# rpng/suo_slam

Measured on AMD Instinct MI355X. Metric: frames/sec (obj-crops/sec) YCB-V 640x480 8-obj; ADD(-S) vs ref, higher is better.
Workload: dtype f32 (2 x fp16 split products)

## Files before the change

### suo_slam_amd/build.py

```python
from __future__ import annotations

import os
import subprocess
import sys

HERE = os.path.dirname(os.path.abspath(__file__))
CSRC = os.path.join(HERE, "csrc")
LIB = os.path.join(HERE, "libsuo_hip.so")
SOURCES = ["capi.hip", "net.hip", "net_weights.hip", "conv.hip", "conv_wino.hip", "conv_wino_x3.hip", "conv_wino_x3_dma.hip", "conv_wino_x3_skip_dma.hip", "conv_small.hip", "stem_x3.hip", "res_small.hip", "res_small_x3.hip", "gemm_persist.hip", "gemm_bf16x3.hip", "misc.hip", "calibrate.hip", "pnp.hip", "lm.hip", "lm_big.hip", "lm_cam.hip", "lm_cam2.hip", "lm_frame.hip", "lm_frame2.hip", "lm_dist.hip", "pose_cov.hip", "pose_cov_graph.hip", "resid_stats.hip", "track_cov.hip", "ba_comm.hip", "pnp_api.hip", "ba_stage.hip", "ba_api.hip", "ba_ctx.hip", "ba_drive.hip", "cov_stage.hip", "pose_cov_api.hip", "track_cov_api.hip", "frame_geom.hip", "eval.hip", "eval_bop.hip", "eval_points.hip", "eval_nees.hip", "eval_nees_api.hip", "raster.hip", "eval_vsd.hip", "gt_info.hip", "gt_info_api.hip", "eval_masks.hip", "slam_score.hip", "slam_vote.hip", "viz.hip", "viz_api.hip"]
HIPCC = os.environ.get("HIPCC", "/opt/rocm/bin/hipcc")
FLAGS = ["--offload-arch=gfx950", "-O3", "-std=c++17", "-fPIC", "-ffp-contract=off"]


def _stale(target, deps):
    if not os.path.exists(target):
        return True
    t = os.path.getmtime(target)
    return any(os.path.getmtime(d) > t for d in deps)


def build(force: bool = False, verbose: bool = True) -> str:
    srcs = [os.path.join(CSRC, s) for s in SOURCES if os.path.exists(os.path.join(CSRC, s))]
    hdrs = [os.path.join(CSRC, f) for f in os.listdir(CSRC) if f.endswith(".h")]
    hdrs.append(os.path.join(os.path.dirname(HERE), "include", "suo_hip.h"))
    objs = []
    procs = []
    for src in srcs:
        obj = src[:-4] + ".o"
        objs.append(obj)
        deps = [src] + hdrs
        if src.endswith("lm_big.hip"):
            deps.append(os.path.join(CSRC, "lm.hip"))
        if force or _stale(obj, deps):
            cmd = [HIPCC] + FLAGS + ["-c", src, "-o", obj]
            if verbose:
                print(" ".join(cmd), flush=True)
            procs.append((src, subprocess.Popen(cmd)))
    for src, p in procs:
        if p.wait() != 0:
            raise RuntimeError(f"hipcc failed on {src}")
    if force or procs or _stale(LIB, objs):
        cmd = [HIPCC, "--offload-arch=gfx950", "-shared", "-fPIC", "-o", LIB] + objs + ["-ldl"]
        if verbose:
            print(" ".join(cmd), flush=True)
        subprocess.check_call(cmd)
    return LIB


if __name__ == "__main__":
    build(force="--force" in sys.argv)
    print(LIB)
```

### suo_slam_amd/csrc/conv_wino_x3_dma.hip

```cpp
#include "conv_wino_x3_kernel.h"

namespace suo {

int launch_conv3x3_wino_f16x2_dma(const ConvArgs& a, hipStream_t s, int tiles) {
    if (a.N == 64) hipLaunchKernelGGL((wino3x3_x3_kernel<false, false, false, 2, 2, false, false, false, true>), dim3(tiles), dim3(256), 0, s, a);
    else hipLaunchKernelGGL((wino3x3_x3_kernel<false, false, false, 4, 2, false, false, false, true>), dim3(tiles), dim3(256), 0, s, a);
    SUO_HIP_CHECK(hipGetLastError());
    return SUO_OK;
}
int launch_conv3x3_wino_f16x2_fused_dma(const ConvArgs& a, hipStream_t s, int tiles) {
    if (a.n_W1) hipLaunchKernelGGL((wino3x3_x3_kernel<true, false, true, 4, 2, true, false, false, true>), dim3(tiles), dim3(256), 0, s, a);
    else if (a.up) hipLaunchKernelGGL((wino3x3_x3_kernel<true, true, true, 4, 2, false, false, false, true>), dim3(tiles), dim3(256), 0, s, a);
    else hipLaunchKernelGGL((wino3x3_x3_kernel<true, false, true, 4, 2, false, false, false, true>), dim3(tiles), dim3(256), 0, s, a);
    SUO_HIP_CHECK(hipGetLastError());
    return SUO_OK;
}

}
```

### suo_slam_amd/csrc/conv_wino_x3_kernel.h

```cpp
#pragma once
#include <string.h>

#include "buffer_ops.h"
#include "mma_ops.h"
#include "suo_internal.h"
#include "tune.h"

namespace suo {

__device__ __forceinline__ f32x4 x_sub4(f32x4 a, f32x4 b) { return a - b; }
__device__ __forceinline__ f32x4 x_add4(f32x4 a, f32x4 b) { return a + b; }
__device__ __forceinline__ void x_add16(f32x16& z, const f32x16& t) { z += t; }
__device__ __forceinline__ void x_sub16(f32x16& z, const f32x16& t) { z -= t; }

constexpr int X_CK = 16, X_PKH = 20, X_TH = 8, X_TW = 16, X_IH = 10, X_IW = 18, X_NPIX = X_IH * X_IW;

template <bool FUSE, bool UP = false, bool TX3 = false, int NT = 4, int NP = 3, bool NEXT = false, bool SKD = false, bool W8 = false, bool DMA = false>
__global__ __launch_bounds__(W8 ? 512 : 256) __attribute__((amdgpu_waves_per_eu(2))) void wino3x3_x3_kernel(const ConvArgs a) {
    static_assert(NT == 4 || (NT == 2 && !FUSE), "64-channel form: plain convolution only");
    static_assert(!DMA || (NP == 2 && !W8), "halo by LDS-DMA: the four-wave fp16 form");
    static_assert(!SKD || (DMA && FUSE && TX3 && UP && !NEXT), "skip rows by LDS-DMA: the LDS-DMA form's tail with the up-sampled addend (the form it measured faster on)");
    static_assert(!W8 || (NT == 4 && NP == 2 && !NEXT && (TX3 || !FUSE)), "eight waves: the fp16 form of the 128-channel kernel, without the next block's conv1");
    constexpr int NTHR = W8 ? 512 : 256;
    static_assert(!NEXT || (FUSE && TX3 && NP == 2), "the next block's conv1 rides on the fp16 tail");
    static_assert(NP == 3 || !FUSE || TX3, "the fp16 form's tail runs on the fp16 pipe");
    constexpr int HSZ = X_NPIX * X_PKH;
    constexpr int VROW = 16;
    constexpr int VPL = 16 * 32 * VROW;
    constexpr int VFLOATS = NP * VPL / 2;
    constexpr int TAILF = NP * 8 * (64 * 32 + 32) / 4;
    constexpr int SKF = SKD ? 4 * 1024 : 0;
    constexpr int SFLOATS = W8 ? (2 * HSZ + VFLOATS > TAILF + 8 * 32 * 36 ? 2 * HSZ + VFLOATS : TAILF + 8 * 32 * 36) : 2 * HSZ + VFLOATS + SKF;
    static_assert(SFLOATS * 4 <= 80 * 1024, "two workgroups per CU");
    __shared__ __attribute__((aligned(16))) float S[SFLOATS];
    float (*Hin)[HSZ] = reinterpret_cast<float (*)[HSZ]>(&S[0]);
    uint16_t* V = reinterpret_cast<uint16_t*>(&S[2 * HSZ]);
    const int tid = threadIdx.x, lane = tid & 63;
    const int w = __builtin_amdgcn_readfirstlane(tid >> 6);
    const int tiles_x = (a.OW + X_TW - 1) / X_TW, tiles_y = (a.OH + X_TH - 1) / X_TH;
    int bid = xcd_block_id();
    const int l = bid / (tiles_x * tiles_y);
    bid -= l * tiles_x * tiles_y;
    const int ty0 = bid / tiles_x, tx0 = bid - ty0 * tiles_x;
    const int oy0 = ty0 * X_TH, ox0 = tx0 * X_TW;
    const int iy0 = oy0 - 1, ix0 = ox0 - 1;
    const int nch = a.C / X_CK;
    const float* in_l = a.in + (size_t)l * a.H * a.W * a.C;
    const __amdgpu_buffer_rsrc_t in_srd = make_srd(in_l, (size_t)a.H * a.W * a.C * sizeof(float));
    const __amdgpu_buffer_rsrc_t w_srd = make_srd(a.Wp, (size_t)a.N * a.C * 16 * NP * sizeof(uint16_t));
    const __amdgpu_buffer_rsrc_t out_srd = make_srd(a.out + (size_t)l * a.OH * a.OW * a.N, (size_t)a.OH * a.OW * a.N * sizeof(float));

    constexpr int NF4 = X_NPIX * 4, NLD = (NF4 + NTHR - 1) / NTHR;
    constexpr int HP = DMA ? 16 : X_PKH;
    static_assert(!DMA || (NLD == 3 && NLD * NTHR * 4 <= HSZ), "LDS-DMA staging: three 1 KiB pieces per wave inside a halo buffer");
    int avoff[NLD];
#pragma unroll
    for (int i = 0; i < NLD; ++i) {
        const int idx = tid + i * NTHR;
        const int pix = idx >> 2;
        const int py = pix / X_IW, px = pix - py * X_IW;
        const int cc = DMA ? (idx & 3) ^ ((py >> 1) & 3) : idx & 3;
        const int iy = iy0 + py, ix = ix0 + px;
        const bool ok = idx < NF4 && iy >= 0 && iy < a.H && ix >= 0 && ix < a.W;
        avoff[i] = ok ? ((iy * a.W + ix) * a.C + cc * 4) * 4 : BUF_OOB;
    }
    const unsigned lds_w = __builtin_amdgcn_readfirstlane((unsigned)(size_t)&S[0]) + w * 1024;
    auto dma = [&](int c, int buf) {
        if constexpr (DMA) {
            const unsigned d0 = lds_w + buf * (HSZ * 4), d1 = d0 + NTHR * 16, d2 = d0 + 2 * NTHR * 16;
            const int soff = c * X_CK * 4;
            unsigned keep;
            asm volatile("s_mov_b32 %0, m0\n\t"
                         "s_nop 4\n\t"
                         "s_mov_b32 m0, %5\n\ts_nop 0\n\tbuffer_load_dwordx4 %1, %4, %8 offen lds\n\t"
                         "s_mov_b32 m0, %6\n\ts_nop 0\n\tbuffer_load_dwordx4 %2, %4, %8 offen lds\n\t"
                         "s_mov_b32 m0, %7\n\ts_nop 0\n\tbuffer_load_dwordx4 %3, %4, %8 offen lds\n\t"
                         "s_mov_b32 m0, %0"
                         : "=&s"(keep)
                         : "v"(avoff[0]), "v"(avoff[NLD > 1 ? 1 : 0]), "v"(avoff[NLD > 2 ? 2 : 0]), "s"(in_srd), "s"(d0), "s"(d1), "s"(d2), "s"(soff)
                         : "memory");
        }
    };
    f32x4 areg[NLD];
    auto gload = [&](int c) {
#pragma unroll
        for (int i = 0; i < NLD; ++i) areg[i] = buf_load(in_srd, avoff[i], c * X_CK * 4);
    };
    float dmax = 0.f;
    const float xs = NP == 2 ? s2_xscale(a.xscale) : 1.f;
    auto sstore = [&](int buf) {
#pragma unroll
        for (int i = 0; i < NLD; ++i) {
            const int idx = tid + i * NTHR;
            if constexpr (NP == 2) {
                areg[i] *= xs;
                dmax = s2_track(s2_track(dmax, areg[i][0], areg[i][1]), areg[i][2], areg[i][3]);
            }
            if (idx < NF4) *(f32x4*)&Hin[buf][(idx >> 2) * X_PKH + (idx & 3) * 4] = areg[i];
        }
    };
    auto dtrack = [&](int buf) {
#pragma unroll
        for (int i = 0; i < NLD; ++i) {
            const f32x4 v = *(const f32x4*)&Hin[buf][(tid + i * NTHR) * 4];
            dmax = s2_track(s2_track(dmax, v[0], v[1]), v[2], v[3]);
        }
    };
    const int wvoff = lane * 16;
    const int wn = NT == 4 ? (W8 ? (w & 3) : w) : (w & 1), wc = NT == 4 ? (W8 ? (w >> 2) : 0) : (w >> 1);
    constexpr bool HALF = NT == 2 || W8;
    constexpr int NPAIR = HALF ? 4 : 8;
    const int wsbase = wn * NP * 1024;
    auto bload = [&](int gc, u32x4 (&b)[NP]) {
        const int g = gc;
#pragma unroll
        for (int p = 0; p < NP; ++p) b[p] = __builtin_bit_cast(u32x4, buf_load(w_srd, wvoff + p * 1024, g * (NT * NP * 1024) + wsbase));
    };
    const int tt = tid & 31, tq = (tid >> 5) & 3, th = (tid >> 7) & 1;
    const int tv = __builtin_amdgcn_readfirstlane(tid >> 8);
    const int t_ty = tt >> 3, t_tx = tt & 7;
    const int hbase = ((2 * t_ty + th) * X_IW + 2 * t_tx) * HP + (DMA ? (tq ^ t_ty) : tq) * 4;
    const int hbase1 = DMA ? ((2 * t_ty + th) * X_IW + 2 * t_tx) * HP + (tq ^ ((t_ty + 1) & 3)) * 4 : hbase;
    const int vbase = tt * VROW + ((((tq >> 1) ^ (((tt >> 2) ^ (tt >> 3)) & 1)) * 8) + (tq & 1) * 4);
    auto vstore = [&](int comp, f32x4 v) {
        if constexpr (NP == 2) {
            split_store4<2, VPL>(&V[comp * 32 * VROW + vbase], v[0], v[1], v[2], v[3]);
            return;
        }
#pragma unroll
        for (int p = 0; p < 3; ++p) {
            const unsigned q0 = s3_pack_rn(v[0], v[1]), q1 = s3_pack_rn(v[2], v[3]);
            *(u32x2*)&V[p * VPL + comp * 32 * VROW + vbase] = u32x2{q0, q1};
            if (p < 2) v = x_sub4(v, f32x4{s3_lo(q0), s3_hi(q0), s3_lo(q1), s3_hi(q1)});
        }
    };
    const int hother = th ? 0 : 2 * X_IW * HP;
    const float hsign = th ? -1.f : 1.f;
    auto transform = [&](int buf) {
        const float* hs = &Hin[buf][hbase];
        if constexpr (W8) {
            const int xi = tv == 0 ? (th ? 3 : 0) : (th ? 2 : 1);
            f32x4 e[4];
#pragma unroll
            for (int c = 0; c < 4; ++c) {
                if (tv == 0) {
                    e[c] = x_sub4(*(const f32x4*)(hs + c * X_PKH), *(const f32x4*)(hs + (2 * X_IW + c) * X_PKH));
                } else {
                    const f32x4 l1 = *(const f32x4*)(hs + (X_IW + c) * X_PKH), lx = *(const f32x4*)(hs + hother + c * X_PKH);
                    e[c] = f32x4{__builtin_fmaf(lx[0], hsign, l1[0]), __builtin_fmaf(lx[1], hsign, l1[1]), __builtin_fmaf(lx[2], hsign, l1[2]), __builtin_fmaf(lx[3], hsign, l1[3])};
                }
            }
            vstore(xi * 4 + 0, x_sub4(e[0], e[2]));
            vstore(xi * 4 + 1, x_add4(e[1], e[2]));
            vstore(xi * 4 + 2, x_sub4(e[2], e[1]));
            vstore(xi * 4 + 3, x_sub4(e[1], e[3]));
            return;
        }
        const float* hs2 = &Hin[buf][hbase1];
        const float* hs1 = th ? hs2 : hs;
        const float* hsx = th ? hs : hs2;
        f32x4 L0[4], L1[4], L2[4], Lx[4];
#pragma unroll
        for (int c = 0; c < 4; ++c) {
            L0[c] = *(const f32x4*)(hs + c * HP);
            L1[c] = *(const f32x4*)(hs1 + (X_IW + c) * HP);
            L2[c] = *(const f32x4*)(hs2 + (2 * X_IW + c) * HP);
            Lx[c] = *(const f32x4*)(hsx + hother + c * HP);
        }
        f32x4 eA[4], eB[4];
#pragma unroll
        for (int c = 0; c < 4; ++c) {
            eA[c] = x_sub4(L0[c], L2[c]);
            eB[c] = f32x4{__builtin_fmaf(Lx[c][0], hsign, L1[c][0]), __builtin_fmaf(Lx[c][1], hsign, L1[c][1]), __builtin_fmaf(Lx[c][2], hsign, L1[c][2]),
                            __builtin_fmaf(Lx[c][3], hsign, L1[c][3])};
            if constexpr (DMA) { eA[c] *= xs; eB[c] *= xs; }
        }
        const int xiA = th ? 3 : 0, xiB = th ? 2 : 1;
        vstore(xiA * 4 + 0, x_sub4(eA[0], eA[2]));
        vstore(xiA * 4 + 1, x_add4(eA[1], eA[2]));
        vstore(xiA * 4 + 2, x_sub4(eA[2], eA[1]));
        vstore(xiA * 4 + 3, x_sub4(eA[1], eA[3]));
        vstore(xiB * 4 + 0, x_sub4(eB[0], eB[2]));
        vstore(xiB * 4 + 1, x_add4(eB[1], eB[2]));
        vstore(xiB * 4 + 2, x_sub4(eB[2], eB[1]));
        vstore(xiB * 4 + 3, x_sub4(eB[1], eB[3]));
    };

    f32x16 zero16;
#pragma unroll
    for (int r = 0; r < 16; ++r) zero16[r] = 0.f;
    f32x16 out[4], Z[8];
#pragma unroll
    for (int p = 0; p < 4; ++p)
#pragma unroll
        for (int r = 0; r < 16; ++r) out[p][r] = 0.f;
#pragma unroll
    for (int p = 0; p < 8; ++p)
#pragma unroll
        for (int r = 0; r < 16; ++r) Z[p][r] = 0.f;
    auto mac6 = [&](f32x16& acc, const bf16x8 (&f)[NP], const u32x4 (&bw)[NP], bool from_zero) {
#pragma unroll
        for (int t = 0; t < split_terms<NP>(); ++t) acc = split_mma<NP>(t, f, bw, (t == 0 && from_zero) ? zero16 : acc);
    };
    auto comp_of = [&](int pair, int which) -> int {
        if (!HALF) return pair < 4 ? (which ? 12 + pair : pair) : (which ? 8 + (pair - 4) : 4 + (pair - 4));
        return wc * 8 + 2 * pair + which;
    };
    const int afoff = (lane & 31) * VROW + (((lane >> 5) ^ (((lane >> 2) ^ (lane >> 3)) & 1)) * 8);
    u32x4 bring[2][2][NP];
    if constexpr (DMA) {
#pragma unroll
        for (int i = 0; i < NLD; ++i)
            if (avoff[i] == BUF_OOB) {
                *(f32x4*)&Hin[0][(tid + i * NTHR) * 4] = f32x4{0.f, 0.f, 0.f, 0.f};
                *(f32x4*)&Hin[1][(tid + i * NTHR) * 4] = f32x4{0.f, 0.f, 0.f, 0.f};
            }
        dma(0, 0);
    } else {
        gload(0);
    }
    bload(comp_of(0, 0), bring[0][0]);
    bload(comp_of(0, 1), bring[0][1]);
    if constexpr (DMA) asm volatile("s_waitcnt vmcnt(0)" ::: "memory");
    else sstore(0);
    __syncthreads();

#ifdef SUO_WX3_PROF
    long long pt[5] = {0, 0, 0, 0, 0}, p0 = clock64();
#define XPROF(i) do { const long long _t = clock64(); pt[i] += _t - p0; p0 = _t; } while (0)
#else
#define XPROF(i) do { } while (0)
#endif
    for (int c = 0; c < nch; ++c) {
        const int buf = c & 1;
        const bool more = c + 1 < nch;
        if (more) {
            if constexpr (DMA) dma(c + 1, buf ^ 1);
            else gload(c + 1);
        }
        transform(buf);
        if constexpr (DMA) dtrack(buf);
        XPROF(0);
        __syncthreads();
        XPROF(1);
        if (more && !DMA) sstore(buf ^ 1);
        XPROF(2);
#pragma unroll
        for (int pair = 0; pair < NPAIR; ++pair) {
            const int slot = pair & 1;
            {
                const int np = pair + 1 < NPAIR ? pair + 1 : 0, nc = pair + 1 < NPAIR ? c : (more ? c + 1 : c);
                bload(nc * 16 + comp_of(np, 0), bring[slot ^ 1][0]);
                bload(nc * 16 + comp_of(np, 1), bring[slot ^ 1][1]);
            }
            const int ca = comp_of(pair, 0), cb = comp_of(pair, 1);
            bf16x8 afa[NP], afb[NP];
#pragma unroll
            for (int p = 0; p < NP; ++p) {
                afa[p] = *(const bf16x8*)&V[p * VPL + ca * 32 * VROW + afoff];
                afb[p] = *(const bf16x8*)&V[p * VPL + cb * 32 * VROW + afoff];
            }
            __builtin_amdgcn_sched_barrier(0);
            if (HALF) {
                mac6(Z[2 * pair], afa, bring[slot][0], false);
                mac6(Z[2 * pair + 1], afb, bring[slot][1], false);
            } else if (pair < 4) {
                mac6(Z[pair], afa, bring[slot][0], false);
                mac6(Z[4 + pair], afb, bring[slot][1], false);
            } else {
                f32x16 ta, tb;
                mac6(ta, afa, bring[slot][0], true);
                mac6(tb, afb, bring[slot][1], true);
                x_add16(Z[pair - 4], ta); x_add16(Z[pair - 4], tb); x_add16(Z[pair], ta); x_sub16(Z[pair], tb);
            }
            __builtin_amdgcn_sched_barrier(0);
        }
        XPROF(3);
        if constexpr (DMA) asm volatile("s_waitcnt vmcnt(4)" ::: "memory");
        __syncthreads();
        XPROF(4);
    }
    if constexpr (DMA) dmax *= xs;
#ifdef SUO_WX3_PROF
    if (blockIdx.x == 1000 && (tid & 63) == 0) printf("wave %d cycles: transform %lld  barrier1 %lld  sstore %lld  mfma+fold %lld  barrier2 %lld\n", w, pt[0], pt[1], pt[2], pt[3], pt[4]);
#endif
    if constexpr (NP == 2) s2_raise(a.range_flag, 4.f * dmax);
#pragma unroll
    for (int h = 0; h < 2; ++h) {
        out[2 * h] = Z[4 * h] + Z[4 * h + 1] + Z[4 * h + 2];
        out[2 * h + 1] = Z[4 * h + 1] - Z[4 * h + 2] - Z[4 * h + 3];
    }
    f32x16 mine[2];
    if constexpr (W8) {
        static_assert(VFLOATS >= 8 * 16 * 64, "the exchange area is the V planes");
        float* X = &S[2 * HSZ];
        const int pw = (1 - wc) * 4 + wn;
#pragma unroll
        for (int q = 0; q < 2; ++q) {
#pragma unroll
            for (int r = 0; r < 16; ++r) X[(w * 16 + r) * 64 + lane] = wc == 0 ? out[2 + q][r] : out[q][r];
            __syncthreads();
#pragma unroll
            for (int r = 0; r < 16; ++r) mine[q][r] = (wc == 0 ? out[q][r] + out[2 + q][r] : out[2 + q][r] - out[q][r]) + X[(pw * 16 + r) * 64 + lane];
            __syncthreads();
        }
    }

    if constexpr (FUSE && TX3) {
        constexpr int KS_STRIDE = 64 * 32 + 32;
        constexpr int PL_STRIDE = 8 * KS_STRIDE;
        static_assert(NP * PL_STRIDE == TAILF * 4 && NP * PL_STRIDE + (W8 ? 8 : 4) * 32 * 36 * 4 <= SFLOATS * 4, "tail staging must fit the workgroup's LDS");
        constexpr int NJ = W8 ? 1 : 2;
        unsigned char* AP = reinterpret_cast<unsigned char*>(&S[0]);
        float* T = &S[NP * PL_STRIDE / 4] + w * (32 * 36);
        const __amdgpu_buffer_rsrc_t w3_srd = make_srd(a.W3p, (size_t)a.N * a.N2 * NP * sizeof(uint16_t));
        const size_t crop2 = (size_t)a.OH * a.OW * a.N2;
        const __amdgpu_buffer_rsrc_t r_srd = make_srd(a.R + (size_t)l * crop2, crop2 * sizeof(float));
        const __amdgpu_buffer_rsrc_t o2_srd = make_srd(a.out2 + (size_t)l * crop2, crop2 * sizeof(float));
        constexpr bool has_up = UP;
        const __amdgpu_buffer_rsrc_t up_srd = make_srd(has_up ? a.up + (size_t)l * (crop2 / 4) : a.R, has_up ? crop2 / 4 * sizeof(float) : 0);
        const float xs3 = NP == 2 ? s2_xscale(a.xscale3) : 1.f;
        const float b2v = NP == 2 ? a.bias[wn * 32 + (lane & 31)] * xs3 : a.bias[wn * 32 + (lane & 31)];
        const float c2v = NP == 2 ? a.oscale[wn * 32 + (lane & 31)] * xs3 : 1.f;
        float tmax = 0.f;
        const int sbase = (2 * wn + ((lane >> 4) & 1)) * KS_STRIDE + (lane >> 5) * (8 * 32) + ((((lane >> 3) & 1) ^ (lane >> 5)) * 16) + (lane & 7) * 2;
        const int aoff = (lane & 31) * 32 + (((lane >> 5) ^ ((lane >> 3) & 1)) * 16);
        const int w3voff = lane * 16;
        const int sk_lane = ((oy0 * a.OW + ox0 + (lane >> 3)) * a.N2 + w * 32 + (lane & 7) * 4) * 4;
        auto skoff = [&](int b, int k) -> int {
            const int row = 2 * (2 * (b & 1) + (k >> 1)) + (b >> 2);
            const int xlim = oy0 + row < a.OH ? a.OW - ox0 - 8 * (k & 1) : 0;
            const int lin = sk_lane + ((row * a.OW + 8 * (k & 1)) * a.N2 + 128 * ((b >> 1) & 1)) * 4;
            return (lane >> 3) < xlim ? lin : BUF_OOB;
        };
        const float* RB = &S[2 * HSZ + VFLOATS] + w * 1024;
        const unsigned rb_w = __builtin_amdgcn_readfirstlane((unsigned)(size_t)&S[2 * HSZ + VFLOATS]) + w * 4096;
        auto skdma = [&](int b, int k) {
            if constexpr (SKD) {
                unsigned keep;
                asm volatile("s_waitcnt lgkmcnt(0)\n\t"
                             "s_mov_b32 %0, m0\n\t"
                             "s_nop 4\n\t"
                             "s_mov_b32 m0, %3\n\ts_nop 0\n\tbuffer_load_dwordx4 %1, %2, 0 offen lds\n\t"
                             "s_mov_b32 m0, %0"
                             : "=&s"(keep)
                             : "v"(skoff(b, k)), "s"(r_srd), "s"(rb_w + k * 1024)
                             : "memory");
            }
        };
        auto skwait = [&](int n) {
            switch (n) {
                case 3: asm volatile("s_waitcnt vmcnt(3)" ::: "memory"); break;
                case 4: asm volatile("s_waitcnt vmcnt(4)" ::: "memory"); break;
                case 5: asm volatile("s_waitcnt vmcnt(5)" ::: "memory"); break;
                case 6: asm volatile("s_waitcnt vmcnt(6)" ::: "memory"); break;
                default: asm volatile("s_waitcnt vmcnt(7)" ::: "memory"); break;
            }
        };
        float* CB = &S[NP * PL_STRIDE / 4 + 4 * 32 * 36];
        if constexpr (SKD) {
            static_assert(NP * PL_STRIDE + 4 * 32 * 36 * 4 + 2 * 256 * 4 <= (2 * HSZ + VFLOATS) * 4 && NTHR == 256, "column vectors: 256 threads, one column each");
            CB[tid] = a.bias3[tid];
            CB[256 + tid] = a.oscale3[tid];
#pragma unroll
            for (int k = 0; k < 4; ++k) skdma(0, k);
        }
        auto b3load = [&](int ks, u32x4 (&b)[2][NP]) {
            const int k = ks < 8 ? ks : 7;
#pragma unroll
            for (int j = 0; j < NJ; ++j)
#pragma unroll
                for (int p = 0; p < NP; ++p) b[j][p] = __builtin_bit_cast(u32x4, buf_load(w3_srd, w3voff, (((k * 8 + (W8 ? w : 4 * j + w)) * NP) + p) * 1024));
        };
#pragma unroll
        for (int h = 0; h < 2; ++h) {
            u32x4 b3[2][2][NP];
            b3load(0, b3[0]);
            if (!W8 || wc == h)
#pragma unroll
            for (int pj = 0; pj < 2; ++pj)
#pragma unroll
                for (int r = 0; r < 16; ++r) {
                    const float cv = W8 ? mine[pj][r] : out[2 * h + pj][r];
                    float v = NP == 2 ? fmaxf(fmaf(cv, c2v, b2v), 0.f) : fmaxf(cv + b2v, 0.f);
                    const int off = sbase + (16 * (r >> 2) + 2 * (r & 3) + pj) * 32;
                    if constexpr (NP == 2) {
                        tmax = fmaxf(tmax, v);
                        const _Float16 hi = (_Float16)v, lo = (_Float16)(v - (float)hi);
                        *reinterpret_cast<_Float16*>(AP + off) = hi;
                        *reinterpret_cast<_Float16*>(AP + PL_STRIDE + off) = lo;
                        continue;
                    }
#pragma unroll
                    for (int p = 0; p < 3; ++p) {
                        const unsigned q = s3_pack_rn(v, v);
                        *reinterpret_cast<uint16_t*>(AP + p * PL_STRIDE + off) = (uint16_t)(q >> 16);
                        if (p < 2) v -= s3_hi(q);
                    }
                }
            __syncthreads();
            f32x16 acc2[2][2];
#pragma unroll
            for (int i = 0; i < 2; ++i)
#pragma unroll
                for (int j = 0; j < 2; ++j)
#pragma unroll
                    for (int r = 0; r < 16; ++r) acc2[i][j][r] = 0.f;
#pragma unroll
            for (int ks = 0; ks < 8; ++ks) {
                b3load(ks + 1, b3[(ks + 1) & 1]);
                bf16x8 af[2][NP];
#pragma unroll
                for (int i = 0; i < 2; ++i)
#pragma unroll
                    for (int p = 0; p < NP; ++p) af[i][p] = *(const bf16x8*)(AP + p * PL_STRIDE + ks * KS_STRIDE + i * 1024 + aoff);
                __builtin_amdgcn_sched_barrier(0);
#pragma unroll
                for (int i = 0; i < 2; ++i)
#pragma unroll
                    for (int j = 0; j < NJ; ++j) mac6(acc2[i][j], af[i], b3[ks & 1][j], false);
                __builtin_amdgcn_sched_barrier(0);
            }
            if constexpr (NEXT) __syncthreads();
            f32x16 acc1[2];
            if constexpr (NEXT) {
#pragma unroll
                for (int i = 0; i < 2; ++i) acc1[i] = zero16;
            }
#pragma unroll
            for (int j = 0; j < NJ; ++j) {
#pragma unroll
                for (int i = 0; i < 2; ++i) {
                    const int col = (W8 ? w : 4 * j + w) * 32 + (lane & 7) * 4;
                    const f32x4 bv = SKD ? *(const f32x4*)&CB[col] : *(const f32x4*)(a.bias3 + col);
                    f32x4 osc3 = f32x4{1.f, 1.f, 1.f, 1.f};
                    if constexpr (NP == 2) osc3 = SKD ? *(const f32x4*)&CB[256 + col] : *(const f32x4*)(a.oscale3 + col);
                    f32x4 nsc, nsh;
                    if constexpr (NEXT) { const float nxs = s2_xscale(a.n_xscale); nsc = *(const f32x4*)(a.n_scale + col) * nxs; nsh = *(const f32x4*)(a.n_shift + col) * nxs; }
                    int off[4];
                    f32x4 rv[SKD ? 1 : 4], uv[UP ? 4 : 1];
#pragma unroll
                    for (int k = 0; k < 4; ++k) {
                        const int m = 32 * i + (lane >> 3) + 8 * k;
                        const int oy = oy0 + 2 * (m >> 4) + h, ox = ox0 + (m & 15);
                        const bool in = oy < a.OH && ox < a.OW;
                        if constexpr (SKD) off[k] = skoff(4 * h + 2 * j + i, k);
                        else off[k] = in ? ((oy * a.OW + ox) * a.N2 + col) * 4 : BUF_OOB;
                        if constexpr (!SKD) rv[k] = buf_load(r_srd, off[k], 0);
                        if constexpr (UP && !NEXT) uv[k] = buf_load(up_srd, in ? (((oy >> 1) * (a.OW >> 1) + (ox >> 1)) * a.N2 + col) * 4 : BUF_OOB, 0);
                    }
#pragma unroll
                    for (int r = 0; r < 16; ++r) T[acc_row(r, lane) * 36 + (lane & 31)] = acc2[i][j][r];
                    __builtin_amdgcn_wave_barrier();
#pragma unroll
                    for (int k = 0; k < 4; ++k) {
                        if constexpr (UP && NEXT) {
                            const int m = 32 * i + (lane >> 3) + 8 * k;
                            const int oy = oy0 + 2 * (m >> 4) + h, ox = ox0 + (m & 15);
                            uv[0] = buf_load(up_srd, (oy < a.OH && ox < a.OW) ? (((oy >> 1) * (a.OW >> 1) + (ox >> 1)) * a.N2 + col) * 4 : BUF_OOB, 0);
                        }
                        f32x4 o = *(const f32x4*)&T[((lane >> 3) + 8 * k) * 36 + (lane & 7) * 4];
                        if constexpr (NP == 2) o *= osc3;
                        if constexpr (SKD) {
                            const int b = 4 * h + 2 * j + i;
                            skwait(b == 0 ? 3 + k : b == 7 ? 7 - k : 7);
                            const f32x4 r = *(const f32x4*)&RB[k * 256 + lane * 4];
                            const bool inmap = off[k] != BUF_OOB;
                            o = (o + bv) + f32x4{inmap ? r[0] : 0.f, inmap ? r[1] : 0.f, inmap ? r[2] : 0.f, inmap ? r[3] : 0.f};
                            if (b < 7) skdma(b + 1, k);
                        } else {
                            o = (o + bv) + rv[k];
                        }
                        if constexpr (UP) o += uv[NEXT ? 0 : k];
                        buf_store(o, o2_srd, off[k]);
                        if constexpr (NEXT) {
                            const int m = 32 * i + (lane >> 3) + 8 * k;
                            float xn[4];
#pragma unroll
                            for (int c = 0; c < 4; ++c) xn[c] = fmaxf(fmaf(o[c], nsc[c], nsh[c]), 0.f);
                            tmax = fmaxf(fmaxf(tmax, fmaxf(xn[0], xn[1])), fmaxf(xn[2], xn[3]));
                            unsigned char* d = AP + (2 * w + ((lane & 7) >> 2)) * KS_STRIDE + m * 32 + (((((lane & 3) >> 1) ^ ((m >> 3) & 1))) * 16) + (lane & 1) * 8;
                            split_store4<2, PL_STRIDE>(d, xn[0], xn[1], xn[2], xn[3]);
                        }
                    }
                    __builtin_amdgcn_wave_barrier();
                }
                if constexpr (NEXT) {
                    const __amdgpu_buffer_rsrc_t n1_srd = make_srd(a.n_W1, (size_t)128 * 256 * 2 * sizeof(uint16_t));
                    auto n1load = [&](int q, u32x4 (&b)[2]) {
                        const int ksg = 8 * j + (q < 8 ? q : 7);
#pragma unroll
                        for (int p = 0; p < 2; ++p) b[p] = __builtin_bit_cast(u32x4, buf_load(n1_srd, w3voff + p * 1024, ((ksg * 4 + w) * 2) * 1024));
                    };
                    constexpr int NR = 4;
                    u32x4 nb[NR][2];
#pragma unroll
                    for (int q = 0; q < NR - 1; ++q) n1load(q, nb[q]);
                    __syncthreads();
#pragma unroll
                    for (int q = 0; q < 8; ++q) {
                        n1load(q + NR - 1, nb[(q + NR - 1) % NR]);
                        bf16x8 af[2][2];
#pragma unroll
                        for (int i = 0; i < 2; ++i)
#pragma unroll
                            for (int p = 0; p < 2; ++p) af[i][p] = *(const bf16x8*)(AP + p * PL_STRIDE + q * KS_STRIDE + i * 1024 + aoff);
                        __builtin_amdgcn_sched_barrier(0);
#pragma unroll
                        for (int i = 0; i < 2; ++i) mac6(acc1[i], af[i], nb[q % NR], false);
                        __builtin_amdgcn_sched_barrier(0);
                    }
                    __syncthreads();
                }
            }
            if constexpr (NEXT) {
                const int col = w * 32 + (lane & 7) * 4;
                const f32x4 b1 = *(const f32x4*)(a.n_b1 + col), o1 = *(const f32x4*)(a.n_osc1 + col);
                const size_t cropn = (size_t)a.OH * a.OW * 128;
                const __amdgpu_buffer_rsrc_t n_srd = make_srd(a.n_out + (size_t)l * cropn, cropn * sizeof(float));
#pragma unroll
                for (int i = 0; i < 2; ++i) {
#pragma unroll
                    for (int r = 0; r < 16; ++r) T[acc_row(r, lane) * 36 + (lane & 31)] = acc1[i][r];
                    __builtin_amdgcn_wave_barrier();
#pragma unroll
                    for (int k = 0; k < 4; ++k) {
                        const int m = 32 * i + (lane >> 3) + 8 * k;
                        const int oy = oy0 + 2 * (m >> 4) + h, ox = ox0 + (m & 15);
                        f32x4 o = *(const f32x4*)&T[((lane >> 3) + 8 * k) * 36 + (lane & 7) * 4];
                        o *= o1;
                        o += b1;
#pragma unroll
                        for (int c = 0; c < 4; ++c) o[c] = fmaxf(o[c], 0.f);
                        buf_store(o, n_srd, (oy < a.OH && ox < a.OW) ? ((oy * a.OW + ox) * 128 + col) * 4 : BUF_OOB);
                    }
                    __builtin_amdgcn_wave_barrier();
                }
            }
            if (h == 0 && !NEXT) __syncthreads();
        }
        if constexpr (NP == 2) s2_raise(a.range_flag, tmax);
        return;
    }

    if constexpr (FUSE && !TX3) {
        constexpr int MP = 132;
        static_assert(128 * MP <= 2 * HSZ + VFLOATS, "the conv2 tile must fit the workgroup's LDS");
        float* M2 = &S[0];
        const int wm = w >> 1, wn = w & 1;
        const int NB2 = a.N2 >> 5;
        const __amdgpu_buffer_rsrc_t w3_srd = make_srd(a.W3p, (size_t)a.N * a.N2 * sizeof(float));
        const size_t crop2 = (size_t)a.OH * a.OW * a.N2;
        const __amdgpu_buffer_rsrc_t r_srd = make_srd(a.R + (size_t)l * crop2, crop2 * sizeof(float));
        const __amdgpu_buffer_rsrc_t o2_srd = make_srd(a.out2 + (size_t)l * crop2, crop2 * sizeof(float));
        constexpr bool has_up = UP;
        const __amdgpu_buffer_rsrc_t up_srd = make_srd(has_up ? a.up + (size_t)l * (crop2 / 4) : a.R, has_up ? crop2 / 4 * sizeof(float) : 0);
        const float b2v = a.bias[w * 32 + (lane & 31)];
        const int w3voff = lane * 16;
        auto b3load = [&](int q, f32x4(&b)[4]) {
            const int kg = q < 16 ? q : 15;
#pragma unroll
            for (int j = 0; j < 4; ++j) b[j] = buf_load(w3_srd, w3voff, (kg * NB2 + wn * 4 + j) * 1024);
        };
        constexpr int R3 = 3;
        f32x4 b3[R3][4];
#pragma unroll
        for (int r = 0; r < R3 - 1; ++r) b3load(r, b3[r]);
#pragma unroll
        for (int p = 0; p < 4; ++p)
#pragma unroll
            for (int r = 0; r < 16; ++r) {
                const int t = acc_row(r, lane);
                const int pix = (2 * (t >> 3) + (p >> 1)) * X_TW + 2 * (t & 7) + (p & 1);
                M2[pix * MP + w * 32 + (lane & 31)] = fmaxf(out[p][r] + b2v, 0.f);
            }
        __syncthreads();
        f32x16 acc2[2][4];
#pragma unroll
        for (int i = 0; i < 2; ++i)
#pragma unroll
            for (int j = 0; j < 4; ++j)
#pragma unroll
                for (int r = 0; r < 16; ++r) acc2[i][j][r] = 0.f;
        const float* ms = M2 + ((wm * 2) * 32 + (lane & 31)) * MP + (lane >> 5) * 4;
#pragma unroll
        for (int q = 0; q < 16; ++q) {
            b3load(q + R3 - 1, b3[(q + R3 - 1) % R3]);
            __builtin_amdgcn_sched_barrier(0);
            f32x4 af[2];
#pragma unroll
            for (int i = 0; i < 2; ++i) af[i] = *(const f32x4*)(ms + i * 32 * MP + q * 8);
#pragma unroll
            for (int t = 0; t < 4; ++t)
#pragma unroll
                for (int i = 0; i < 2; ++i)
#pragma unroll
                    for (int j = 0; j < 4; ++j) acc2[i][j] = mfma32(af[i][t], b3[q % R3][j][t], acc2[i][j]);
            __builtin_amdgcn_sched_barrier(0);
        }
        __syncthreads();
#pragma unroll
        for (int i = 0; i < 2; ++i)
#pragma unroll
            for (int j = 0; j < 4; ++j) {
                float* T = M2 + w * (32 * 36);
                const int col = (wn * 4 + j) * 32 + (lane & 7) * 4;
                const f32x4 bv = *(const f32x4*)(a.bias3 + col);
                int off[4];
                f32x4 rv[4], uv[UP ? 4 : 1];
#pragma unroll
                for (int k = 0; k < 4; ++k) {
                    const int pp = (wm * 2 + i) * 32 + (lane >> 3) + 8 * k;
                    const int oy = oy0 + pp / X_TW, ox = ox0 + pp % X_TW;
                    const bool in = oy < a.OH && ox < a.OW;
                    off[k] = in ? ((oy * a.OW + ox) * a.N2 + col) * 4 : BUF_OOB;
                    rv[k] = buf_load(r_srd, off[k], 0);
                    if constexpr (UP) uv[k] = buf_load(up_srd, in ? (((oy >> 1) * (a.OW >> 1) + (ox >> 1)) * a.N2 + col) * 4 : BUF_OOB, 0);
                }
#pragma unroll
                for (int r = 0; r < 16; ++r) T[acc_row(r, lane) * 36 + (lane & 31)] = acc2[i][j][r];
                __builtin_amdgcn_wave_barrier();
#pragma unroll
                for (int k = 0; k < 4; ++k) {
                    f32x4 o = (*(const f32x4*)&T[((lane >> 3) + 8 * k) * 36 + (lane & 7) * 4] + bv) + rv[k];
                    if constexpr (UP) o += uv[k];
                    buf_store(o, o2_srd, off[k]);
                }
                __builtin_amdgcn_wave_barrier();
            }
        return;
    }

    if constexpr (NT == 2 || W8) {
        if constexpr (NT == 2) {
            float* X = &S[2 * HSZ];
#pragma unroll
            for (int q = 0; q < 2; ++q)
#pragma unroll
                for (int r = 0; r < 16; ++r) X[((w * 2 + q) * 16 + r) * 64 + lane] = wc == 0 ? out[2 + q][r] : out[q][r];
            __syncthreads();
            const int pw = (1 - wc) * 2 + wn;
#pragma unroll
            for (int q = 0; q < 2; ++q)
#pragma unroll
                for (int r = 0; r < 16; ++r)
                    mine[q][r] = (wc == 0 ? out[q][r] + out[2 + q][r] : out[2 + q][r] - out[q][r]) + X[((pw * 2 + q) * 16 + r) * 64 + lane];
            __syncthreads();
        }
        float* T = &S[2 * HSZ] + w * (32 * 36);
        const int col = wn * 32 + (lane & 7) * 4;
        const f32x4 bv = *(const f32x4*)(a.bias + col);
        f32x4 osc = f32x4{1.f, 1.f, 1.f, 1.f};
        if constexpr (NP == 2) osc = *(const f32x4*)(a.oscale + col);
#pragma unroll
        for (int q = 0; q < 2; ++q) {
            const int p = 2 * wc + q, pi = p >> 1, pj = p & 1;
#pragma unroll
            for (int r = 0; r < 16; ++r) T[acc_row(r, lane) * 36 + (lane & 31)] = mine[q][r];
            __builtin_amdgcn_wave_barrier();
#pragma unroll
            for (int k = 0; k < 4; ++k) {
                const int t = (lane >> 3) + 8 * k;
                const int oy = oy0 + 2 * (t >> 3) + pi, ox = ox0 + 2 * (t & 7) + pj;
                f32x4 o = *(const f32x4*)&T[t * 36 + (lane & 7) * 4];
                if constexpr (NP == 2) o *= osc;
                o += bv;
                if (a.relu) {
#pragma unroll
                    for (int z = 0; z < 4; ++z) o[z] = fmaxf(o[z], 0.f);
                }
                buf_store(o, out_srd, (oy < a.OH && ox < a.OW) ? ((oy * a.OW + ox) * a.N + col) * 4 : BUF_OOB);
            }
            __builtin_amdgcn_wave_barrier();
        }
        return;
    }

    float* T = &S[2 * HSZ] + w * (32 * 36);
    const int col = w * 32 + (lane & 7) * 4;
    const f32x4 bv = *(const f32x4*)(a.bias + col);
    f32x4 osc = f32x4{1.f, 1.f, 1.f, 1.f};
    if constexpr (NP == 2) osc = *(const f32x4*)(a.oscale + col);
#pragma unroll
    for (int p = 0; p < 4; ++p) {
        const int pi = p >> 1, pj = p & 1;
#pragma unroll
        for (int r = 0; r < 16; ++r) T[acc_row(r, lane) * 36 + (lane & 31)] = out[p][r];
        __builtin_amdgcn_wave_barrier();
#pragma unroll
        for (int k = 0; k < 4; ++k) {
            const int t = (lane >> 3) + 8 * k;
            const int oy = oy0 + 2 * (t >> 3) + pi, ox = ox0 + 2 * (t & 7) + pj;
            f32x4 o = *(const f32x4*)&T[t * 36 + (lane & 7) * 4];
            if constexpr (NP == 2) o *= osc;
            o += bv;
            if (a.relu) {
#pragma unroll
                for (int q = 0; q < 4; ++q) o[q] = fmaxf(o[q], 0.f);
            }
            buf_store(o, out_srd, (oy < a.OH && ox < a.OW) ? ((oy * a.OW + ox) * a.N + col) * 4 : BUF_OOB);
        }
        __builtin_amdgcn_wave_barrier();
    }
}

}
```

### suo_slam_amd/csrc/conv_wino_x3_skip_dma.hip

```cpp
#include "conv_wino_x3_kernel.h"

namespace suo {

int launch_conv3x3_wino_f16x2_fused_up_skip_dma(const ConvArgs& a, hipStream_t s, int tiles) {
    hipLaunchKernelGGL((wino3x3_x3_kernel<true, true, true, 4, 2, false, true, false, true>), dim3(tiles), dim3(256), 0, s, a);
    SUO_HIP_CHECK(hipGetLastError());
    return SUO_OK;
}

}
```

### suo_slam_amd/csrc/tune.h

```cpp
#pragma once
#include <stdlib.h>

namespace suo {
inline long env_switch(const char* name, long dflt) {
    const char* e = getenv(name);
    return e ? atol(e) : dflt;
}
inline bool env_set(const char* name) { return getenv(name) != nullptr; }
}

#ifdef SUO_TUNING
#define SUO_TUNE(name, dflt) suo::env_switch(name, (long)(dflt))
#else
#define SUO_TUNE(name, dflt) ((long)(dflt))
#endif
```

Before: 1440.

## Overlap Winograd output-transform fold with next pair's MFMAs in fp16 DMA kernels

Adds a fold-overlap variant of the four-wave fp16 LDS-DMA Winograd kernel. It reorders the channel-component pairs so the add/sub fold of one pair's MFMA results is interleaved with the next pair's MFMAs, using sched_group_barrier hints and optional asm pinning of the fold adds. The goal is to hide the VALU fold latency behind matrix-core work in the inner loop. The variant is on by default through an environment switch and routes the plain, fused and skip-DMA launchers to it. It also reworks the profiling hooks. Holding the extra fta/ftb live across pairs raises register pressure.

Result: no change. 1425 (-1.0%).

```diff
diff --git a/suo_slam_amd/build.py b/suo_slam_amd/build.py
--- a/suo_slam_amd/build.py
+++ b/suo_slam_amd/build.py
@@ -7,7 +7,7 @@
 HERE = os.path.dirname(os.path.abspath(__file__))
 CSRC = os.path.join(HERE, "csrc")
 LIB = os.path.join(HERE, "libsuo_hip.so")
-SOURCES = ["capi.hip", "net.hip", "net_weights.hip", "conv.hip", "conv_wino.hip", "conv_wino_x3.hip", "conv_wino_x3_dma.hip", "conv_wino_x3_skip_dma.hip", "conv_small.hip", "stem_x3.hip", "res_small.hip", "res_small_x3.hip", "gemm_persist.hip", "gemm_bf16x3.hip", "misc.hip", "calibrate.hip", "pnp.hip", "lm.hip", "lm_big.hip", "lm_cam.hip", "lm_cam2.hip", "lm_frame.hip", "lm_frame2.hip", "lm_dist.hip", "pose_cov.hip", "pose_cov_graph.hip", "resid_stats.hip", "track_cov.hip", "ba_comm.hip", "pnp_api.hip", "ba_stage.hip", "ba_api.hip", "ba_ctx.hip", "ba_drive.hip", "cov_stage.hip", "pose_cov_api.hip", "track_cov_api.hip", "frame_geom.hip", "eval.hip", "eval_bop.hip", "eval_points.hip", "eval_nees.hip", "eval_nees_api.hip", "raster.hip", "eval_vsd.hip", "gt_info.hip", "gt_info_api.hip", "eval_masks.hip", "slam_score.hip", "slam_vote.hip", "viz.hip", "viz_api.hip"]
+SOURCES = ["capi.hip", "net.hip", "net_weights.hip", "conv.hip", "conv_wino.hip", "conv_wino_x3.hip", "conv_wino_x3_dma.hip", "conv_wino_x3_skip_dma.hip", "conv_wino_x3_fold.hip", "conv_small.hip", "stem_x3.hip", "res_small.hip", "res_small_x3.hip", "gemm_persist.hip", "gemm_bf16x3.hip", "misc.hip", "calibrate.hip", "pnp.hip", "lm.hip", "lm_big.hip", "lm_cam.hip", "lm_cam2.hip", "lm_frame.hip", "lm_frame2.hip", "lm_dist.hip", "pose_cov.hip", "pose_cov_graph.hip", "resid_stats.hip", "track_cov.hip", "ba_comm.hip", "pnp_api.hip", "ba_stage.hip", "ba_api.hip", "ba_ctx.hip", "ba_drive.hip", "cov_stage.hip", "pose_cov_api.hip", "track_cov_api.hip", "frame_geom.hip", "eval.hip", "eval_bop.hip", "eval_points.hip", "eval_nees.hip", "eval_nees_api.hip", "raster.hip", "eval_vsd.hip", "gt_info.hip", "gt_info_api.hip", "eval_masks.hip", "slam_score.hip", "slam_vote.hip", "viz.hip", "viz_api.hip"]
 HIPCC = os.environ.get("HIPCC", "/opt/rocm/bin/hipcc")
 FLAGS = ["--offload-arch=gfx950", "-O3", "-std=c++17", "-fPIC", "-ffp-contract=off"]
 
diff --git a/suo_slam_amd/csrc/conv_wino_x3_dma.hip b/suo_slam_amd/csrc/conv_wino_x3_dma.hip
--- a/suo_slam_amd/csrc/conv_wino_x3_dma.hip
+++ b/suo_slam_amd/csrc/conv_wino_x3_dma.hip
@@ -2,13 +2,19 @@
 
 namespace suo {
 
+bool conv3x3_wino_f16x2_fold_overlap();
+int launch_conv3x3_wino_f16x2_fold(const ConvArgs& a, hipStream_t s, int tiles);
+int launch_conv3x3_wino_f16x2_fused_fold(const ConvArgs& a, hipStream_t s, int tiles, bool skip_dma);
+
 int launch_conv3x3_wino_f16x2_dma(const ConvArgs& a, hipStream_t s, int tiles) {
+    if (a.N != 64 && conv3x3_wino_f16x2_fold_overlap()) return launch_conv3x3_wino_f16x2_fold(a, s, tiles);
     if (a.N == 64) hipLaunchKernelGGL((wino3x3_x3_kernel<false, false, false, 2, 2, false, false, false, true>), dim3(tiles), dim3(256), 0, s, a);
     else hipLaunchKernelGGL((wino3x3_x3_kernel<false, false, false, 4, 2, false, false, false, true>), dim3(tiles), dim3(256), 0, s, a);
     SUO_HIP_CHECK(hipGetLastError());
     return SUO_OK;
 }
 int launch_conv3x3_wino_f16x2_fused_dma(const ConvArgs& a, hipStream_t s, int tiles) {
+    if (conv3x3_wino_f16x2_fold_overlap()) return launch_conv3x3_wino_f16x2_fused_fold(a, s, tiles, false);
     if (a.n_W1) hipLaunchKernelGGL((wino3x3_x3_kernel<true, false, true, 4, 2, true, false, false, true>), dim3(tiles), dim3(256), 0, s, a);
     else if (a.up) hipLaunchKernelGGL((wino3x3_x3_kernel<true, true, true, 4, 2, false, false, false, true>), dim3(tiles), dim3(256), 0, s, a);
     else hipLaunchKernelGGL((wino3x3_x3_kernel<true, false, true, 4, 2, false, false, false, true>), dim3(tiles), dim3(256), 0, s, a);
diff --git a/suo_slam_amd/csrc/conv_wino_x3_fold.hip b/suo_slam_amd/csrc/conv_wino_x3_fold.hip
--- /dev/null
+++ b/suo_slam_amd/csrc/conv_wino_x3_fold.hip
@@ -0,0 +1,48 @@
+#include "conv_wino_x3_kernel.h"
+
+namespace suo {
+
+#ifdef SUO_WX3_PROF
+bool conv3x3_wino_f16x2_fold_overlap() { return true; }
+static bool prof_old_order() { return env_switch("SUO_WINO_FOLD_OVERLAP", 1) == 0; }
+#else
+bool conv3x3_wino_f16x2_fold_overlap() { return env_switch("SUO_WINO_FOLD_OVERLAP", 1) != 0; }
+#endif
+
+int launch_conv3x3_wino_f16x2_fold(const ConvArgs& a, hipStream_t s, int tiles) {
+#ifdef SUO_WX3_PROF
+    if (prof_old_order()) hipLaunchKernelGGL((wino3x3_x3_kernel<false, false, false, 4, 2, false, false, false, true>), dim3(tiles), dim3(256), 0, s, a);
+    else
+#endif
+    hipLaunchKernelGGL((wino3x3_x3_fold_kernel<false>), dim3(tiles), dim3(256), 0, s, a);
+    SUO_HIP_CHECK(hipGetLastError());
+    return SUO_OK;
+}
+int launch_conv3x3_wino_f16x2_fused_fold(const ConvArgs& a, hipStream_t s, int tiles, bool skip_dma) {
+#ifdef SUO_WX3_PROF
+    if (prof_old_order()) {
+        if (a.n_W1) hipLaunchKernelGGL((wino3x3_x3_kernel<true, false, true, 4, 2, true, false, false, true>), dim3(tiles), dim3(256), 0, s, a);
+        else if (a.up && skip_dma) hipLaunchKernelGGL((wino3x3_x3_kernel<true, true, true, 4, 2, false, true, false, true>), dim3(tiles), dim3(256), 0, s, a);
+        else if (a.up) hipLaunchKernelGGL((wino3x3_x3_kernel<true, true, true, 4, 2, false, false, false, true>), dim3(tiles), dim3(256), 0, s, a);
+        else hipLaunchKernelGGL((wino3x3_x3_kernel<true, false, true, 4, 2, false, false, false, true>), dim3(tiles), dim3(256), 0, s, a);
+        SUO_HIP_CHECK(hipGetLastError());
+        return SUO_OK;
+    }
+#endif
+    if (a.n_W1) hipLaunchKernelGGL((wino3x3_x3_fold_kernel<true, false, true>), dim3(tiles), dim3(256), 0, s, a);
+    else if (a.up && skip_dma) hipLaunchKernelGGL((wino3x3_x3_fold_kernel<true, true, false, true>), dim3(tiles), dim3(256), 0, s, a);
+    else if (a.up) hipLaunchKernelGGL((wino3x3_x3_fold_kernel<true, true>), dim3(tiles), dim3(256), 0, s, a);
+    else hipLaunchKernelGGL((wino3x3_x3_fold_kernel<true>), dim3(tiles), dim3(256), 0, s, a);
+    SUO_HIP_CHECK(hipGetLastError());
+    return SUO_OK;
+}
+
+#ifdef SUO_WX3_PROF
+extern "C" int suo_wx3_prof_read(long long* out) {
+    SUO_HIP_CHECK(hipDeviceSynchronize());
+    SUO_HIP_CHECK(hipMemcpyFromSymbol(out, HIP_SYMBOL(x_prof_buf), sizeof(long long) * 64));
+    return SUO_OK;
+}
+#endif
+
+}
diff --git a/suo_slam_amd/csrc/conv_wino_x3_kernel.h b/suo_slam_amd/csrc/conv_wino_x3_kernel.h
--- a/suo_slam_amd/csrc/conv_wino_x3_kernel.h
+++ b/suo_slam_amd/csrc/conv_wino_x3_kernel.h
@@ -12,12 +12,45 @@
 __device__ __forceinline__ f32x4 x_add4(f32x4 a, f32x4 b) { return a + b; }
 __device__ __forceinline__ void x_add16(f32x16& z, const f32x16& t) { z += t; }
 __device__ __forceinline__ void x_sub16(f32x16& z, const f32x16& t) { z -= t; }
+template <bool PL>
+__device__ __forceinline__ void x_fold_add(f32x16& z, const f32x16& t, bool sub) {
+    if constexpr (PL) {
+#pragma unroll
+        for (int r = 0; r < 16; ++r) {
+            float v = sub ? z[r] - t[r] : z[r] + t[r];
+            asm("" : "+v"(v));
+            z[r] = v;
+        }
+    } else {
+        if (sub) x_sub16(z, t);
+        else x_add16(z, t);
+    }
+}
+template <int PART, bool PL>
+__device__ __forceinline__ void x_fold(f32x16& z0, f32x16& z1, const f32x16& ta, const f32x16& tb) {
+    if (PART != 2) { x_fold_add<PL>(z0, ta, false); x_fold_add<PL>(z1, ta, false); x_fold_add<PL>(z0, tb, false); }
+    if (PART != 1) x_fold_add<PL>(z1, tb, true);
+}
+template <bool PL>
+constexpr int x_fold_gap(bool scratch) { return scratch ? 6 : PL ? (SUO_WX3_FOLD_SPREAD ? 8 : 11) : (SUO_WX3_FOLD_SPREAD ? 7 : 6); }
+#ifdef SUO_WX3_PROF
+#ifndef SUO_WX3_PROF_BLOCK
+#define SUO_WX3_PROF_BLOCK 1000
+#endif
+static __device__ long long x_prof_buf[8 * 8];
+#endif
+#define X_FOLD_GAP(n)                                              \
+    do {                                                           \
+        __builtin_amdgcn_sched_group_barrier(0x008, 1, 0);         \
+        __builtin_amdgcn_sched_group_barrier(0x002, n, 0);         \
+    } while (0)
 
 constexpr int X_CK = 16, X_PKH = 20, X_TH = 8, X_TW = 16, X_IH = 10, X_IW = 18, X_NPIX = X_IH * X_IW;
 
-template <bool FUSE, bool UP = false, bool TX3 = false, int NT = 4, int NP = 3, bool NEXT = false, bool SKD = false, bool W8 = false, bool DMA = false>
-__global__ __launch_bounds__(W8 ? 512 : 256) __attribute__((amdgpu_waves_per_eu(2))) void wino3x3_x3_kernel(const ConvArgs a) {
+template <bool FUSE, bool UP, bool TX3, int NT, int NP, bool NEXT, bool SKD, bool W8, bool DMA, bool FO>
+__device__ __forceinline__ void wino3x3_x3_body(const ConvArgs& a) {
     static_assert(NT == 4 || (NT == 2 && !FUSE), "64-channel form: plain convolution only");
+    static_assert(!FO || (NT == 4 && NP == 2 && !W8), "fold under the next pair's MFMAs: the four-wave fp16 forms that fold");
     static_assert(!DMA || (NP == 2 && !W8), "halo by LDS-DMA: the four-wave fp16 form");
     static_assert(!SKD || (DMA && FUSE && TX3 && UP && !NEXT), "skip rows by LDS-DMA: the LDS-DMA form's tail with the up-sampled addend (the form it measured faster on)");
     static_assert(!W8 || (NT == 4 && NP == 2 && !NEXT && (TX3 || !FUSE)), "eight waves: the fp16 form of the 128-channel kernel, without the next block's conv1");
@@ -203,6 +236,7 @@
         for (int t = 0; t < split_terms<NP>(); ++t) acc = split_mma<NP>(t, f, bw, (t == 0 && from_zero) ? zero16 : acc);
     };
     auto comp_of = [&](int pair, int which) -> int {
+        if (FO) return pair & 1 ? (which ? 8 + (pair >> 1) : 4 + (pair >> 1)) : (which ? 12 + (pair >> 1) : pair >> 1);
         if (!HALF) return pair < 4 ? (which ? 12 + pair : pair) : (which ? 8 + (pair - 4) : 4 + (pair - 4));
         return wc * 8 + 2 * pair + which;
     };
@@ -226,7 +260,7 @@
     __syncthreads();
 
 #ifdef SUO_WX3_PROF
-    long long pt[5] = {0, 0, 0, 0, 0}, p0 = clock64();
+    long long pt[6] = {0, 0, 0, 0, 0, 0}, p0 = clock64();
 #define XPROF(i) do { const long long _t = clock64(); pt[i] += _t - p0; p0 = _t; } while (0)
 #else
 #define XPROF(i) do { } while (0)
@@ -245,6 +279,9 @@
         XPROF(1);
         if (more && !DMA) sstore(buf ^ 1);
         XPROF(2);
+        f32x16 fta, ftb;
+        constexpr bool FPL = SUO_WX3_FOLD_PLAIN == 2 || (SUO_WX3_FOLD_PLAIN == 1 && FUSE);
+        constexpr int FGD = x_fold_gap<FPL>(false), FGS = x_fold_gap<FPL>(true);
 #pragma unroll
         for (int pair = 0; pair < NPAIR; ++pair) {
             const int slot = pair & 1;
@@ -264,6 +301,25 @@
             if (HALF) {
                 mac6(Z[2 * pair], afa, bring[slot][0], false);
                 mac6(Z[2 * pair + 1], afb, bring[slot][1], false);
+            } else if constexpr (FO) {
+                const int nu = pair >> 1;
+                if (!(pair & 1)) {
+                    mac6(Z[nu], afa, bring[slot][0], false);
+                    mac6(Z[4 + nu], afb, bring[slot][1], false);
+                    if (nu > 0) {
+                        x_fold<SUO_WX3_FOLD_SPREAD ? 1 : 0, FPL>(Z[nu - 1], Z[3 + nu], fta, ftb);
+                        X_FOLD_GAP(FGD); X_FOLD_GAP(FGD); X_FOLD_GAP(FGD); X_FOLD_GAP(FGD); X_FOLD_GAP(FGD); X_FOLD_GAP(FGD);
+                    }
+                } else {
+                    mac6(fta, afa, bring[slot][0], true);
+                    if (SUO_WX3_FOLD_SPREAD && nu > 0) {
+                        x_fold<2, FPL>(Z[nu - 1], Z[3 + nu], fta, ftb);
+                        X_FOLD_GAP(FGS); X_FOLD_GAP(FGS); X_FOLD_GAP(FGS);
+                    }
+                    mac6(ftb, afb, bring[slot][1], true);
+                    if (pair + 1 < NPAIR) { XPROF(5); continue; }
+                    x_fold<0, FPL>(Z[nu], Z[4 + nu], fta, ftb);
+                }
             } else if (pair < 4) {
                 mac6(Z[pair], afa, bring[slot][0], false);
                 mac6(Z[4 + pair], afb, bring[slot][1], false);
@@ -274,15 +330,16 @@
                 x_add16(Z[pair - 4], ta); x_add16(Z[pair - 4], tb); x_add16(Z[pair], ta); x_sub16(Z[pair], tb);
             }
             __builtin_amdgcn_sched_barrier(0);
-        }
-        XPROF(3);
+            XPROF((HALF || (FO ? !(pair & 1) : pair < 4)) ? 3 : 5);
+        }
         if constexpr (DMA) asm volatile("s_waitcnt vmcnt(4)" ::: "memory");
         __syncthreads();
         XPROF(4);
     }
     if constexpr (DMA) dmax *= xs;
 #ifdef SUO_WX3_PROF
-    if (blockIdx.x == 1000 && (tid & 63) == 0) printf("wave %d cycles: transform %lld  barrier1 %lld  sstore %lld  mfma+fold %lld  barrier2 %lld\n", w, pt[0], pt[1], pt[2], pt[3], pt[4]);
+    if (blockIdx.x == SUO_WX3_PROF_BLOCK && lane == 0)
+        for (int i = 0; i < 6; ++i) x_prof_buf[w * 8 + i] = pt[i];
 #endif
     if constexpr (NP == 2) s2_raise(a.range_flag, 4.f * dmax);
 #pragma unroll
@@ -704,4 +761,13 @@
     }
 }
 
+template <bool FUSE, bool UP = false, bool TX3 = false, int NT = 4, int NP = 3, bool NEXT = false, bool SKD = false, bool W8 = false, bool DMA = false>
+__global__ __launch_bounds__(W8 ? 512 : 256) __attribute__((amdgpu_waves_per_eu(2))) void wino3x3_x3_kernel(const ConvArgs a) {
+    wino3x3_x3_body<FUSE, UP, TX3, NT, NP, NEXT, SKD, W8, DMA, false>(a);
 }
+template <bool FUSE, bool UP = false, bool NEXT = false, bool SKD = false>
+__global__ __launch_bounds__(256) __attribute__((amdgpu_waves_per_eu(2))) void wino3x3_x3_fold_kernel(const ConvArgs a) {
+    wino3x3_x3_body<FUSE, UP, FUSE, 4, 2, NEXT, SKD, false, true, true>(a);
+}
+
+}
diff --git a/suo_slam_amd/csrc/conv_wino_x3_skip_dma.hip b/suo_slam_amd/csrc/conv_wino_x3_skip_dma.hip
--- a/suo_slam_amd/csrc/conv_wino_x3_skip_dma.hip
+++ b/suo_slam_amd/csrc/conv_wino_x3_skip_dma.hip
@@ -2,7 +2,11 @@
 
 namespace suo {
 
+bool conv3x3_wino_f16x2_fold_overlap();
+int launch_conv3x3_wino_f16x2_fused_fold(const ConvArgs& a, hipStream_t s, int tiles, bool skip_dma);
+
 int launch_conv3x3_wino_f16x2_fused_up_skip_dma(const ConvArgs& a, hipStream_t s, int tiles) {
+    if (conv3x3_wino_f16x2_fold_overlap()) return launch_conv3x3_wino_f16x2_fused_fold(a, s, tiles, true);
     hipLaunchKernelGGL((wino3x3_x3_kernel<true, true, true, 4, 2, false, true, false, true>), dim3(tiles), dim3(256), 0, s, a);
     SUO_HIP_CHECK(hipGetLastError());
     return SUO_OK;
diff --git a/suo_slam_amd/csrc/tune.h b/suo_slam_amd/csrc/tune.h
--- a/suo_slam_amd/csrc/tune.h
+++ b/suo_slam_amd/csrc/tune.h
@@ -9,6 +9,13 @@
 inline bool env_set(const char* name) { return getenv(name) != nullptr; }
 }
 
+#ifndef SUO_WX3_FOLD_PLAIN
+#define SUO_WX3_FOLD_PLAIN 1
+#endif
+#ifndef SUO_WX3_FOLD_SPREAD
+#define SUO_WX3_FOLD_SPREAD 1
+#endif
+
 #ifdef SUO_TUNING
 #define SUO_TUNE(name, dflt) suo::env_switch(name, (long)(dflt))
 #else
```
